# ross39/new_bloom_filter_repo

Hardware: AMD Instinct MI355X
Metric: Mpixels/s Bloom insert+query, 1080p residuals (higher is better)
Workload: dtype u64

## Files before the change

new_bloom_filter_repo_amd/csrc/rbf_kernels_insert_f64.h:

```cpp
#pragma once
#include "rbf_f64_common.h"
#include "rbf_kernels.h"
#include "rbf_lds_dma.h"

namespace rbf {

constexpr int HT_THREADS = 256;

__global__ __launch_bounds__(HT_THREADS) void k_hash_table(uint64_t n, Seeds seeds, uint4 *__restrict__ table)
{
    const uint32_t lane = threadIdx.x & 63u, wave = threadIdx.x >> 6;
    const uint64_t seg = (uint64_t)blockIdx.x * (HT_THREADS / WAVE) + wave;
    if (seg * QL_SEG_PIXELS >= n) return;
    const uint64_t i0 = seg * QL_SEG_PIXELS + (uint64_t)lane * QL_P;
    uint64_t h1[QL_P], h2[QL_P], ha[QL_P];
    uint32_t validmask = 0;
#pragma unroll
    for (int it = 0; it < QL_P; ++it) {
        h1[it] = 0; h2[it] = 0; ha[it] = 0;
        if (i0 + it < n) validmask |= 1u << it;
    }
    if (!hash3_run8((uint32_t)i0, validmask, seeds, h1, h2, ha)) {
#pragma unroll
        for (int it = 0; it < QL_P; ++it) {
            const bool act = (validmask >> it) & 1u;
            const Hash3 h = hash3_index((uint32_t)(i0 + it), act, seeds);
            h1[it] = h.h1; h2[it] = h.h2; ha[it] = h.ha;
        }
    }
    hash_table_store8(table, n, seg, lane, h1, h2, ha);
}

static_assert(IT_WAVE_LDS_BYTES % 16 == 0 && (IT_QUEUE * 2) % 16 == 0, "the stage is written by LDS-DMA");

template <bool RECORDS, int NWAVES, bool HASHED = false, bool WHOLE = false>
__device__ __forceinline__ void insert_tab_steps(const uint8_t *__restrict__ mask , uint64_t row_bytes , uint64_t n,
                                                 const FrameDev &fd, const uint4 *__restrict__ table, const Seeds &seeds,
                                                 uint32_t *filt, uint32_t tile_bit0, uint32_t tile_bits, uint2 *__restrict__ records, uint32_t rpos,
                                                 uint32_t *wave_lds , uint64_t g0, uint64_t g1, uint32_t lane, uint32_t wave)
{
    static_assert((NWAVES & (NWAVES - 1)) == 0, "a power of two");
    uint16_t *q = reinterpret_cast<uint16_t *>(wave_lds);
    const uint32_t stage = __builtin_amdgcn_readfirstlane(lds_addr_of(wave_lds) + IT_QUEUE * 2);
    uint32_t qn = 0;
    const uint32_t m = vgpr_copy(__builtin_amdgcn_readfirstlane(fd.m));
    const uint32_t fk = __builtin_amdgcn_readfirstlane(fd.floor_k);
    const double ninv = __builtin_bit_cast(double, fd.M);
    const uint64_t T = fd.T;
    auto set_bit = [&](uint32_t pos) {
        if (WHOLE) { atomicOr(&filt[pos >> 5], msb_bit(pos)); return; }
        const uint32_t rel = pos - tile_bit0;
        if (rel < tile_bits) atomicOr(&filt[rel >> 5], msb_bit(pos));
    };

    const HashTable tv(const_cast<uint4 *>(table), n);
    const uint32_t Ttag = (uint32_t)(T >> 48);
    uint4 e0 = make_uint4(0, 0, 0, 0);
    uint32_t tag = 0, slot_kept = 0;
    uint64_t ha_kept = 0;
    uint32_t pending = 0;
    uint32_t cb = 0;
    auto fetch = [&](uint32_t first, uint32_t count) {
        const uint32_t e = lane < count ? q[first + lane] : 0u;
        const uint32_t idx = ((cb + (e >> 10) * NWAVES) << 10) + (e & 1023u);
        if (HASHED) {
            const Hash3 h = hash3_index(idx, lane < count, seeds);
            e0 = make_uint4((uint32_t)h.h1, (uint32_t)(h.h1 >> 32), (uint32_t)h.h2, (uint32_t)(h.h2 >> 32));
            tag = (uint32_t)(h.ha >> 48);
            ha_kept = h.ha;
        } else {
            slot_kept = hash_table_slot(idx);
            e0 = tv.pos[slot_kept];
            tag = tv.tag[idx];
        }
        pending = count;
    };
    auto finish = [&]() {
        if (!pending) return;
        if (lane < pending) {
            uint32_t pos = mod_m_f64(rn_double(e0.x, e0.y), e0.x, ninv, m);
            const uint32_t step = mod_m_f64(rn_double(e0.z, e0.w), e0.z, ninv, m);
            bool act = tag < Ttag;
            if (tag == Ttag) act = (HASHED ? ha_kept : tv.act[slot_kept]) < T;
            if (RECORDS) {
                records[rpos + lane] = make_uint2(pos, step | (act ? 0x80000000u : 0u));
            } else {
                for (uint32_t j = 0; j < fk; ++j) {
                    set_bit(pos);
                    const uint32_t s2 = pos + step;
                    pos = min(s2, s2 - m);
                }
                if (act) set_bit(pos);
            }
        }
        if (RECORDS) rpos += pending;
        pending = 0;
    };

    const uint32_t nbytes32 = (uint32_t)((n + 7) >> 3), n32 = (uint32_t)n, row32 = (uint32_t)row_bytes;
    const uint32_t gend = (uint32_t)g1;
    auto staged = [&](uint32_t s) -> uint32_t {
        return *reinterpret_cast<const __attribute__((address_space(3))) uint16_t *>((uintptr_t)(stage + s * IT_STEP_BYTES + lane * 2u));
    };
    auto decode = [&](uint32_t v, uint32_t g) -> uint32_t {
        const uint32_t byte = g * IT_STEP_BYTES + lane * 2u;
        const uint32_t x = __builtin_bitreverse32(v) >> 16;
        uint32_t b = ((x & 0xFFu) << 8) | (x >> 8);
        const uint32_t rem = n32 - byte * 8u;
        if (rem < 16u) b &= (1u << rem) - 1u;
        return (g < gend && byte < nbytes32) ? b : 0u;
    };
    for (uint32_t chunk = __builtin_amdgcn_readfirstlane((uint32_t)g0 + wave); chunk < gend; chunk += NWAVES * IT_CHUNK_STEPS) {
        cb = chunk;
        wave_lds_fence();
#pragma unroll
        for (int i = 0; i < IT_CHUNK_STEPS / 2; ++i) {
            const uint32_t g = cb + (2u * i + (lane >> 5)) * NWAVES;
            const uint32_t off = g * IT_STEP_BYTES + (lane & 31u) * 4u;
            if (g < gend && off < row32) {
                const uint32_t dst = stage + (uint32_t)i * 256u;
                uint32_t keep;
                asm volatile("s_mov_b32 %0, m0\n\ts_mov_b32 m0, %1\n\ts_nop 0\n\tglobal_load_lds_dword %2, %3\n\ts_mov_b32 m0, %0"
                             : "=&s"(keep) : "s"(dst), "v"(off), "s"(mask) : "memory");
            }
        }
        dma_wait_all();
        wave_lds_fence();
        uint32_t nxt = staged(0);
        for (uint32_t s = 0; s < IT_CHUNK_STEPS && cb + s * NWAVES < gend; ++s) {
            const uint32_t g = cb + s * NWAVES;
            uint32_t bits = decode(nxt, g);
            nxt = staged(s + 1 < IT_CHUNK_STEPS ? s + 1 : s);
            const uint32_t c = __popc(bits);
            const uint32_t incl = wave_inclusive_scan(c);
            const uint32_t excl = incl - c;
            const uint32_t total = __builtin_amdgcn_readlane(incl, 63);
            uint32_t off = qn + excl;
            const uint32_t ebase = (s << 10) | (lane << 4);
            while (bits) {
                q[off++] = (uint16_t)(ebase + __builtin_ctz(bits));
                bits &= bits - 1u;
            }
            qn += total;
            wave_lds_fence();
            while (qn >= WAVE) {
                qn -= WAVE;
                finish();
                fetch(qn, WAVE);
            }
            wave_lds_fence();
        }
        if (cb + NWAVES * IT_CHUNK_STEPS < gend && qn) {
            finish();
            fetch(0, qn);
            qn = 0;
            wave_lds_fence();
        }
    }
    finish();
    if (qn) { fetch(0, qn); finish(); }
}

template <bool HASHED = false, bool WHOLE = false>
__global__ __launch_bounds__(IL_THREADS) void k_insert_tab(
    const uint8_t *__restrict__ masks, uint64_t mask_stride_bytes, uint64_t n,
    const FrameTable tab, const uint4 *__restrict__ table , Seeds seeds,
    uint32_t *__restrict__ partials, uint64_t part_stride_words32, uint32_t tile_words ,
    const SliceTable slices, uint32_t per_tile , uint32_t Smax )
{
    extern __shared__ __attribute__((aligned(16))) uint32_t lds[];
    uint32_t *filt = lds;
    uint32_t *queues = lds + tile_words;
    const uint32_t tile = blockIdx.x / per_tile;
    uint32_t s = blockIdx.x - tile * per_tile, f = 0;
    while (s >= slices.n[f]) { s -= slices.n[f]; ++f; }
    const uint32_t S = slices.n[f];
    const FrameDev fd = tab.f[f];
    if (fd.m == 0) return;
    const uint32_t lane = threadIdx.x & 63u, wave = threadIdx.x >> 6;
    const uint32_t fwords = filter_words(fd.m);
    const uint32_t tile0 = tile * tile_words;
    if (tile0 >= fwords) return;
    for (uint32_t i = threadIdx.x; i < tile_words; i += IL_THREADS) filt[i] = 0;
    __syncthreads();

    const uint64_t nbytes = (n + 7) >> 3;
    const uint64_t groups = (nbytes + IT_STEP_BYTES - 1) / IT_STEP_BYTES;
    const uint64_t gper = (groups + S - 1) / S;
    const uint64_t g0 = (uint64_t)s * gper;
    const uint64_t g1 = g0 + gper < groups ? g0 + gper : groups;
    insert_tab_steps<false, IL_WAVES, HASHED, WHOLE>(masks + (uint64_t)f * mask_stride_bytes, mask_stride_bytes, n, fd, table, seeds, filt, tile0 << 5, tile_words << 5, nullptr, 0u,
                                                     queues + wave * (IT_WAVE_LDS_BYTES / 4), g0, g1, lane, wave);
    __syncthreads();
    uint32_t *part = partials + ((uint64_t)f * Smax + s) * part_stride_words32 + tile0;
    const uint32_t mine = fwords - tile0 < tile_words ? fwords - tile0 : tile_words;
    const uint32_t pairs = (mine + 1) >> 1;
    for (uint32_t i = threadIdx.x; i < pairs; i += IL_THREADS)
        reinterpret_cast<uint2 *>(part)[i] = reinterpret_cast<const uint2 *>(filt)[i];
}

constexpr int IP_THREADS = 256, IP_WAVES = IP_THREADS / WAVE;

template <bool HASHED = false>
__global__ __launch_bounds__(IP_THREADS) void k_insert_positions(
    const uint8_t *__restrict__ masks, uint64_t mask_stride_bytes, uint64_t n,
    const FrameTable tab , const uint4 *__restrict__ table , Seeds seeds,
    uint2 *__restrict__ records, uint32_t *__restrict__ counters )
{
    __shared__ __attribute__((aligned(16))) uint32_t queues[IP_WAVES * (IT_WAVE_LDS_BYTES / 4)];
    const uint32_t f = blockIdx.y, s = blockIdx.x, S = gridDim.x;
    const FrameDev fd = tab.f[f];
    if (fd.m == 0) return;
    const uint32_t lane = threadIdx.x & 63u, wave = threadIdx.x >> 6;
    const uint64_t nbytes = (n + 7) >> 3;
    const uint64_t groups = (nbytes + IT_STEP_BYTES - 1) / IT_STEP_BYTES;
    const uint64_t gper = (groups + S - 1) / S;
    const uint64_t g0 = (uint64_t)s * gper;
    const uint64_t g1 = g0 + gper < groups ? g0 + gper : groups;
    const uint8_t *mask = masks + (uint64_t)f * mask_stride_bytes;
    __shared__ uint32_t wcount[IP_WAVES];
    __shared__ uint32_t wg_base;
    uint32_t mine = 0;
    for (uint64_t g = g0 + wave; g < g1; g += IP_WAVES) {
        const uint64_t byte = g * IT_STEP_BYTES + lane * 2;
        if (byte < nbytes) {
            uint32_t v = *reinterpret_cast<const uint16_t *>(mask + byte);
            const uint64_t rem = n - byte * 8;
            if (rem < 16) {
                const uint32_t x = __builtin_bitreverse32(v) >> 16;
                v = (((x & 0xFFu) << 8) | (x >> 8)) & ((1u << rem) - 1u);
            }
            mine += __popc(v);
        }
    }
    const uint32_t wave_total = __builtin_amdgcn_readlane(wave_inclusive_scan(mine), 63);
    if (lane == 0) wcount[wave] = wave_total;
    __syncthreads();
    if (threadIdx.x == 0) {
        uint32_t t = 0;
        for (int k = 0; k < IP_WAVES; ++k) t += wcount[k];
        wg_base = t ? atomicAdd(counters + f, t) : 0u;
    }
    __syncthreads();
    uint32_t rpos = wg_base;
    for (uint32_t k = 0; k < wave; ++k) rpos += wcount[k];
    insert_tab_steps<true, IP_WAVES, HASHED>(mask, mask_stride_bytes, n, fd, table, seeds, nullptr, 0u, 0u, records + fd.floor_k, (uint32_t)__builtin_amdgcn_readfirstlane((int)rpos),
                                             queues + wave * (IT_WAVE_LDS_BYTES / 4), g0, g1, lane, wave);
}

constexpr int IR_UNROLL = 4;

__global__ __launch_bounds__(IL_THREADS) void k_insert_records(
    const uint2 *__restrict__ records, const uint32_t *__restrict__ counters, const FrameTable tab ,
    uint32_t *__restrict__ partials, uint64_t part_stride_words32, uint32_t tile_words ,
    const SliceTable slices, uint32_t per_tile , uint32_t Smax)
{
    extern __shared__ __attribute__((aligned(16))) uint32_t lds[];
    const uint32_t tile = blockIdx.x / per_tile;
    uint32_t s = blockIdx.x - tile * per_tile, f = 0;
    while (s >= slices.n[f]) { s -= slices.n[f]; ++f; }
    const uint32_t S = slices.n[f];
    const uint32_t m = tab.f[f].m;
    if (m == 0) return;
    const uint32_t fk = tab.f[f].floor_k;
    const uint32_t fwords = filter_words(m);
    const uint32_t tile0 = tile * tile_words;
    if (tile0 >= fwords) return;
    const uint32_t tile_bit0 = tile0 << 5, tile_bits = tile_words << 5;
    for (uint32_t i = threadIdx.x; i < tile_words; i += IL_THREADS) lds[i] = 0;
    __syncthreads();
    const uint32_t count = counters[f];
    const uint32_t per = (((count + S - 1) / S) + 63u) & ~63u;
    const uint32_t r0 = s * per < count ? s * per : count, r1 = r0 + per < count ? r0 + per : count;
    const uint2 *rec = records + tab.f[f].T;
    auto insert = [&](uint2 r) {
        uint32_t pos = r.x;
        const uint32_t step = r.y & 0x7FFFFFFFu;
        for (uint32_t j = 0; j < fk; ++j) {
            const uint32_t rel = pos - tile_bit0;
            if (rel < tile_bits) atomicOr(&lds[rel >> 5], msb_bit(pos));
            const uint32_t s2 = pos + step;
            pos = min(s2, s2 - m);
        }
        const uint32_t rel = pos - tile_bit0;
        if ((r.y >> 31) && rel < tile_bits) atomicOr(&lds[rel >> 5], msb_bit(pos));
    };
    uint32_t i = r0 + threadIdx.x;
    for (; i + (IR_UNROLL - 1) * IL_THREADS < r1; i += IR_UNROLL * IL_THREADS) {
        uint2 r[IR_UNROLL];
#pragma unroll
        for (int u = 0; u < IR_UNROLL; ++u) r[u] = rec[i + u * IL_THREADS];
#pragma unroll
        for (int u = 0; u < IR_UNROLL; ++u) insert(r[u]);
    }
    for (; i < r1; i += IL_THREADS) insert(rec[i]);
    __syncthreads();
    uint32_t *part = partials + ((uint64_t)f * Smax + s) * part_stride_words32 + tile0;
    const uint32_t mine = fwords - tile0 < tile_words ? fwords - tile0 : tile_words;
    const uint32_t pairs = (mine + 1) >> 1;
    for (uint32_t k = threadIdx.x; k < pairs; k += IL_THREADS)
        reinterpret_cast<uint2 *>(part)[k] = reinterpret_cast<const uint2 *>(lds)[k];
}

}
```

new_bloom_filter_repo_amd/csrc/rbf_query_f64_pass.h:

```cpp
#pragma once
#include "rbf_f64_common.h"

namespace rbf {

#define RBF_ROW() __builtin_amdgcn_sched_barrier(0)

__device__ __forceinline__ void rows_reduce4(int g, const double (&hd1)[QL_P], const uint32_t (&hl1)[QL_P], const double (&hd2)[QL_P], const uint32_t (&hl2)[QL_P],
                                             uint32_t m , double ninv, uint32_t (&x)[4])
{
    const int i0 = 2 * g, i1 = 2 * g + 1;
    const double t0 = __builtin_fma(hd1[i0], ninv, 0x1.8p52), t1 = __builtin_fma(hd2[i0], ninv, 0x1.8p52);
    const double t2 = __builtin_fma(hd1[i1], ninv, 0x1.8p52), t3 = __builtin_fma(hd2[i1], ninv, 0x1.8p52);
    RBF_ROW();
    const uint32_t s0 = (uint32_t)__builtin_bit_cast(uint64_t, t0) * m + hl1[i0], s1 = (uint32_t)__builtin_bit_cast(uint64_t, t1) * m + hl2[i0];
    const uint32_t s2 = (uint32_t)__builtin_bit_cast(uint64_t, t2) * m + hl1[i1], s3 = (uint32_t)__builtin_bit_cast(uint64_t, t3) * m + hl2[i1];
    RBF_ROW();
    const uint32_t q0 = s0 + m, q1 = s1 + m, q2 = s2 + m, q3 = s3 + m;
    RBF_ROW();
    x[0] = min(s0, q0); x[1] = min(s1, q1); x[2] = min(s2, q2); x[3] = min(s3, q3);
    RBF_ROW();
}

template <int FK, bool OVERLAP = true, bool PRIO = true, typename STAGER, typename HOOK>
__device__ __forceinline__ void frame_pass_rows(
    const double (&hd1)[QL_P], const uint32_t (&hl1)[QL_P], const double (&hd2)[QL_P], const uint32_t (&hl2)[QL_P],
    uint32_t rank_lo, uint32_t rank_hi, uint32_t c , uint32_t lds_base_bytes , uint32_t safe_pos , uint32_t m , double ninv,
    uint32_t (&x)[4], uint32_t &pbf, STAGER &st, HOOK &&after_first_reads)
{
    static_assert(FK >= 1, "at least one deterministic probe");
    constexpr int NP = FK + 1, NG = QL_P / 2;
    uint32_t pos[OVERLAP ? 2 : 1][2][NP], wrd[OVERLAP ? 2 : 1][2][NP];
    uint32_t five = 5u;
    asm volatile("" : "+s"(five));
    auto lds_word = [&](uint32_t addr) -> uint32_t { return *reinterpret_cast<const __attribute__((address_space(3))) uint32_t *>((uintptr_t)addr); };
    auto steps_and_reads = [&](int g, const uint32_t (&x)[4]) {
        const int par = OVERLAP ? g & 1 : 0;
        uint32_t pa = x[0], pb_ = x[2];
        const uint32_t sa = x[1], sb = x[3];
#pragma unroll
        for (int j = 0; j < FK; ++j) {
            pos[par][0][j] = pa; pos[par][1][j] = pb_;
            const uint32_t wa = pa >> five, wb = pb_ >> five;
            const uint32_t ua = pa + sa, ub = pb_ + sb;
            RBF_ROW();
            const uint32_t aa = (wa << 2) + lds_base_bytes, ab = (wb << 2) + lds_base_bytes;
            const uint32_t va = ua - m, vb = ub - m;
            RBF_ROW();
            wrd[par][0][j] = lds_word(aa); wrd[par][1][j] = lds_word(ab);
            pa = min(ua, va); pb_ = min(ub, vb);
            RBF_ROW();
        }
        const int i0 = 2 * g, i1 = 2 * g + 1;
        const uint32_t rk0 = i0 < 4 ? rank_lo : rank_hi, rk1 = i1 < 4 ? rank_lo : rank_hi;
        uint64_t k0, k1;
        if ((i0 & 3) == 0) { k0 = rank_le<0>(rk0, c); k1 = rank_le<1>(rk1, c); }
        else { k0 = rank_le<2>(rk0, c); k1 = rank_le<3>(rk1, c); }
        RBF_ROW();
        pos[par][0][FK] = select_by(k0, safe_pos, pa); pos[par][1][FK] = select_by(k1, safe_pos, pb_);
        RBF_ROW();
        const uint32_t wa = pos[par][0][FK] >> five, wb = pos[par][1][FK] >> five;
        RBF_ROW();
        const uint32_t aa = (wa << 2) + lds_base_bytes, ab = (wb << 2) + lds_base_bytes;
        RBF_ROW();
        wrd[par][0][FK] = lds_word(aa); wrd[par][1][FK] = lds_word(ab);
        RBF_ROW();
    };
    auto combine2 = [&](int g) {
        const int par = OVERLAP ? g & 1 : 0;
        uint32_t f0 = 0u, f1 = 0u;
        __builtin_amdgcn_s_waitcnt(0xC07F);
#pragma unroll
        for (int j = 0; j < NP; ++j) {
            f0 = (wrd[par][0][j] << (pos[par][0][j] & 31u)) | f0;
            f1 = (wrd[par][1][j] << (pos[par][1][j] & 31u)) | f1;
            RBF_ROW();
        }
        pbf = __builtin_amdgcn_alignbit(pbf, f0, 31);
        RBF_ROW();
        pbf = __builtin_amdgcn_alignbit(pbf, f1, 31);
        RBF_ROW();
    };
    if (PRIO) __builtin_amdgcn_s_setprio(3);
    steps_and_reads(0, x);
    st.at(0);
    RBF_ROW();
    after_first_reads();
    RBF_ROW();
#pragma unroll
    for (int g = 1; g < NG; ++g) {
        if (PRIO) { if (g == 1) __builtin_amdgcn_s_setprio(2); else if (g == 2) __builtin_amdgcn_s_setprio(1); else __builtin_amdgcn_s_setprio(0); }
        rows_reduce4(g, hd1, hl1, hd2, hl2, m, ninv, x);
        combine2(g - 1);
        steps_and_reads(g, x);
        st.at(g);
        RBF_ROW();
    }
    combine2(NG - 1);
    st.at(4);
}

template <typename STAGER>
__device__ __forceinline__ void frame_pass_plain(
    const double (&hd1)[QL_P], const uint32_t (&hl1)[QL_P], const double (&hd2)[QL_P], const uint32_t (&hl2)[QL_P],
    uint32_t rank_lo, uint32_t rank_hi, uint32_t c, uint32_t validmask, uint32_t lds_base_bytes, uint32_t safe_pos, uint32_t m, double ninv,
    uint32_t fk, uint32_t &pbf, STAGER &st)
{
#pragma unroll
    for (int it = 0; it < QL_P; ++it) {
        if ((it & 1) == 0) st.at(it >> 1);
        uint32_t pos = mod_m_f64(hd1[it], hl1[it], ninv, m);
        const uint32_t step = mod_m_f64(hd2[it], hl2[it], ninv, m);
        uint32_t fail = ~(validmask << (31 - it)) & 0x80000000u;
        for (uint32_t j = 0; j < fk; ++j) {
            fail = (probe_image_word(lds_base_bytes, pos) << (pos & 31u)) | fail;
            const uint32_t s2 = pos + step;
            pos = min(s2, s2 - m);
        }
        const uint32_t rk = ((it < 4 ? rank_lo : rank_hi) >> (8 * (it & 3))) & 0xFFu;
        const uint32_t pc = rk <= c ? pos : safe_pos;
        fail = (probe_image_word(lds_base_bytes, pc) << (pc & 31u)) | fail;
        pbf = __builtin_amdgcn_alignbit(pbf, fail, 31);
    }
    st.at(4);
}

#undef RBF_ROW

}
```

Before: 557,800.

## Decode staged mask bits as 32-bit words with tail masking and queue split

The insert scan now reads 32-bit words from the LDS stage and walks two steps per iteration, dropping the per-lane bitreverse/byteswap decode. Instead, element indices are remapped with an XOR-7 in fetch, and a tail mask is applied only near the end of the row. Because one iteration can now enqueue up to twice as many bits, the queue push is split in halves when it would overflow. The query pass swaps the opaque SGPR shift amount for an inline v_lshrrev with an immediate 5. The bit-ordering remap and the split-queue logic add risk of index mistakes.

```diff
diff --git a/new_bloom_filter_repo_amd/csrc/rbf_kernels_insert_f64.h b/new_bloom_filter_repo_amd/csrc/rbf_kernels_insert_f64.h
--- a/new_bloom_filter_repo_amd/csrc/rbf_kernels_insert_f64.h
+++ b/new_bloom_filter_repo_amd/csrc/rbf_kernels_insert_f64.h
@@ -61,8 +61,8 @@
     uint32_t pending = 0;
     uint32_t cb = 0;
     auto fetch = [&](uint32_t first, uint32_t count) {
-        const uint32_t e = lane < count ? q[first + lane] : 0u;
-        const uint32_t idx = ((cb + (e >> 10) * NWAVES) << 10) + (e & 1023u);
+        const uint32_t e = lane < count ? q[first + lane] : 7u;
+        const uint32_t idx = ((cb + (e >> 10) * NWAVES) << 10) + ((e & 1023u) ^ 7u);
         if (HASHED) {
             const Hash3 h = hash3_index(idx, lane < count, seeds);
             e0 = make_uint4((uint32_t)h.h1, (uint32_t)(h.h1 >> 32), (uint32_t)h.h2, (uint32_t)(h.h2 >> 32));
@@ -97,18 +97,19 @@
         pending = 0;
     };
 
-    const uint32_t nbytes32 = (uint32_t)((n + 7) >> 3), n32 = (uint32_t)n, row32 = (uint32_t)row_bytes;
+    const uint32_t n32 = (uint32_t)n, row32 = (uint32_t)row_bytes;
     const uint32_t gend = (uint32_t)g1;
+    const uint32_t gwhole = min(gend, n32 >> 10);
+    const uint32_t pair_addr = stage + lane * 4u, lane_e = lane << 5;
     auto staged = [&](uint32_t s) -> uint32_t {
-        return *reinterpret_cast<const __attribute__((address_space(3))) uint16_t *>((uintptr_t)(stage + s * IT_STEP_BYTES + lane * 2u));
-    };
-    auto decode = [&](uint32_t v, uint32_t g) -> uint32_t {
-        const uint32_t byte = g * IT_STEP_BYTES + lane * 2u;
-        const uint32_t x = __builtin_bitreverse32(v) >> 16;
-        uint32_t b = ((x & 0xFFu) << 8) | (x >> 8);
-        const uint32_t rem = n32 - byte * 8u;
-        if (rem < 16u) b &= (1u << rem) - 1u;
-        return (g < gend && byte < nbytes32) ? b : 0u;
+        return *reinterpret_cast<const __attribute__((address_space(3))) uint32_t *>((uintptr_t)(pair_addr + s * IT_STEP_BYTES));
+    };
+    auto tail_mask = [&](uint32_t s) -> uint32_t {
+        const uint32_t g = cb + (s + (lane >> 5)) * NWAVES;
+        const uint32_t rem = n32 - (g << 10), first = (lane & 31u) << 5;
+        if (g >= gend || rem <= first) return 0u;
+        const uint32_t natural = rem - first >= 32u ? ~0u : (1u << (rem - first)) - 1u;
+        return __builtin_bswap32(__builtin_bitreverse32(natural));
     };
     for (uint32_t chunk = __builtin_amdgcn_readfirstlane((uint32_t)g0 + wave); chunk < gend; chunk += NWAVES * IT_CHUNK_STEPS) {
         cb = chunk;
@@ -127,28 +128,34 @@
         dma_wait_all();
         wave_lds_fence();
         uint32_t nxt = staged(0);
-        for (uint32_t s = 0; s < IT_CHUNK_STEPS && cb + s * NWAVES < gend; ++s) {
-            const uint32_t g = cb + s * NWAVES;
-            uint32_t bits = decode(nxt, g);
-            nxt = staged(s + 1 < IT_CHUNK_STEPS ? s + 1 : s);
+        for (uint32_t s = 0; s < IT_CHUNK_STEPS && cb + s * NWAVES < gend; s += 2) {
+            uint32_t bits = nxt;
+            if (cb + (s + 1) * NWAVES >= gwhole) bits &= tail_mask(s);
+            nxt = staged(s + 2 < IT_CHUNK_STEPS ? s + 2 : s);
             const uint32_t c = __popc(bits);
             const uint32_t incl = wave_inclusive_scan(c);
             const uint32_t excl = incl - c;
             const uint32_t total = __builtin_amdgcn_readlane(incl, 63);
-            uint32_t off = qn + excl;
-            const uint32_t ebase = (s << 10) | (lane << 4);
-            while (bits) {
-                q[off++] = (uint16_t)(ebase + __builtin_ctz(bits));
-                bits &= bits - 1u;
+            const uint32_t ebase = (s << 10) + lane_e;
+            const bool split = qn + total > IT_QUEUE;
+            const uint32_t first = split ? __builtin_amdgcn_readlane(incl, 31) : total;
+            uint32_t part = split && lane >= 32u ? 0u : bits, off = qn + excl, count = first;
+            for (bool more = split;; more = false) {
+                while (part) {
+                    q[off++] = (uint16_t)(ebase + __builtin_ctz(part));
+                    part &= part - 1u;
+                }
+                qn += count;
+                wave_lds_fence();
+                while (qn >= WAVE) {
+                    qn -= WAVE;
+                    finish();
+                    fetch(qn, WAVE);
+                }
+                wave_lds_fence();
+                if (!more) break;
+                part = lane >= 32u ? bits : 0u; off = qn + excl - first; count = total - first;
             }
-            qn += total;
-            wave_lds_fence();
-            while (qn >= WAVE) {
-                qn -= WAVE;
-                finish();
-                fetch(qn, WAVE);
-            }
-            wave_lds_fence();
         }
         if (cb + NWAVES * IT_CHUNK_STEPS < gend && qn) {
             finish();
diff --git a/new_bloom_filter_repo_amd/csrc/rbf_query_f64_pass.h b/new_bloom_filter_repo_amd/csrc/rbf_query_f64_pass.h
--- a/new_bloom_filter_repo_amd/csrc/rbf_query_f64_pass.h
+++ b/new_bloom_filter_repo_amd/csrc/rbf_query_f64_pass.h
@@ -30,8 +30,7 @@
     static_assert(FK >= 1, "at least one deterministic probe");
     constexpr int NP = FK + 1, NG = QL_P / 2;
     uint32_t pos[OVERLAP ? 2 : 1][2][NP], wrd[OVERLAP ? 2 : 1][2][NP];
-    uint32_t five = 5u;
-    asm volatile("" : "+s"(five));
+    auto word_of = [](uint32_t pos) -> uint32_t { uint32_t w; asm("v_lshrrev_b32 %0, 5, %1" : "=v"(w) : "v"(pos)); return w; };
     auto lds_word = [&](uint32_t addr) -> uint32_t { return *reinterpret_cast<const __attribute__((address_space(3))) uint32_t *>((uintptr_t)addr); };
     auto steps_and_reads = [&](int g, const uint32_t (&x)[4]) {
         const int par = OVERLAP ? g & 1 : 0;
@@ -40,7 +39,7 @@
 #pragma unroll
         for (int j = 0; j < FK; ++j) {
             pos[par][0][j] = pa; pos[par][1][j] = pb_;
-            const uint32_t wa = pa >> five, wb = pb_ >> five;
+            const uint32_t wa = word_of(pa), wb = word_of(pb_);
             const uint32_t ua = pa + sa, ub = pb_ + sb;
             RBF_ROW();
             const uint32_t aa = (wa << 2) + lds_base_bytes, ab = (wb << 2) + lds_base_bytes;
@@ -58,7 +57,7 @@
         RBF_ROW();
         pos[par][0][FK] = select_by(k0, safe_pos, pa); pos[par][1][FK] = select_by(k1, safe_pos, pb_);
         RBF_ROW();
-        const uint32_t wa = pos[par][0][FK] >> five, wb = pos[par][1][FK] >> five;
+        const uint32_t wa = word_of(pos[par][0][FK]), wb = word_of(pos[par][1][FK]);
         RBF_ROW();
         const uint32_t aa = (wa << 2) + lds_base_bytes, ab = (wb << 2) + lds_base_bytes;
         RBF_ROW();
```

After: 556,700. About the same (-0.2%).
